# UNC-CFD/somar

Measured on AMD Instinct MI355X. Metric: pressure-Poisson V-cycles/sec, higher is better.
Workload: dtype f64; 1 GPU; C2 single-level 512^3 Poisson, diagonal stretched metric, Neumann, LevelGSRB V-cycle 2/2/2 + BiCGStab bottom; layout = 1 box(es) 512x512x512, one per GPU; mg_depth=8, cells=134217728

## Files before the change

### somar_amd/csrc/gsrb_fused.hip

```cpp
#include <type_traits>

#include "common.h"
#include "kernels.h"
#include "stencil_point.h"

namespace somar {


template <class T>
__device__ __forceinline__ typename Vec2<T>::type uni2(double c, bool, bool) { return mk2<T>(T(c), T(c)); }

template <int FR_J, int INMODE, bool DIRI, bool UNI, bool INT, int CLS, class T>
__device__ __forceinline__ void gsrb_fused_body(T* __restrict__ S, const Tile& t, const PatchDesc& p,
                                                T* __restrict__ phi_out,
                                                const T* __restrict__ phi_in,
                                                const T* __restrict__ rhs,
                                                const T* __restrict__ jgx,
                                                const T* __restrict__ jgy,
                                                const T* __restrict__ jgz,
                                                const T* __restrict__ jinv, const StencilParams& P,
                                                const double* __restrict__ sums,
                                                const PatchDesc* __restrict__ cpatches,
                                                const T* __restrict__ crse, int r0, int r1, int r2)
{
    typedef typename Vec2<T>::type T2;
    const T avg = (INMODE == 2 || INMODE == 4) ? T(sums[0] / sums[1]) : T(0);
    constexpr int LPR = 64 >> CLS;
    constexpr int NR = FR_J << CLS;
    constexpr int PITCH = 2 * LPR + (CLS >= 2 ? 2 : 0);
#define Sx(slot, r, c) S[((slot) * NR + (r)) * PITCH + (c)]
    const int lane = CLS == 0 ? (int)threadIdx.x : (int)(threadIdx.x & (LPR - 1));
    const int row = CLS == 0 ? (int)threadIdx.y
                             : (int)(((threadIdx.y >> 1) << (CLS + 1)) + (threadIdx.y & 1) + 2 * (threadIdx.x >> (6 - CLS)));
    const int ri = 2 * lane;
    const int li = t.i0 - 2 + ri;
    const int wi = t.w > 0 ? t.w : 2 * LPR - 4;
    const int lj = t.j0 - 2 + row;
    long long cbase = 0, cpk = 0, coff = 0;
    int cstep = 0, csh2 = 0;
    if (INMODE >= 3) {
        const PatchDesc cp = cpatches[t.patch];
        auto fdiv = [](int a, int b) { return a >= 0 ? a / b : -((-a + b - 1) / b); };
        const int ci0 = fdiv(li, r0);
        cstep = fdiv(li + 1, r0) - ci0;
        coff = cp.off;
        cbase = cp.off + ci0 + (long long)cp.pj * fdiv(lj, r1);
        cpk = cp.pk;
        csh2 = r2 >> 1;
    }
    auto ldphi = [&](int kp, bool ok0, bool ok1) {
        if (INMODE == 1) return mk2<T>(T(0), T(0));
        T2 v = ld2(phi_in, p.off + li + (long long)p.pj * lj + p.pk * kp, ok0, ok1, p.off);
        if (INMODE >= 3) {
            const bool any = ok0 || ok1;
            const long long c = any ? cbase + cpk * (long long)(kp >> csh2) : coff;
            const long long c2 = any ? c + cstep : coff;
            const T c0 = crse[c];
            const T c1 = crse[c2];
            v.x = ok0 ? v.x + c0 : T(0);
            v.y = ok1 ? v.y + c1 : T(0);
        }
        if (INMODE == 2 || INMODE == 4) { v.x = v.x - avg; v.y = v.y - avg; }
        return v;
    };
    const int gj = p.lo[1] + lj;
    const T xxS = T(1.0) / (T(P.dx[0]) * T(P.dx[0]));
    const T yyS = T(1.0) / (T(P.dx[1]) * T(P.dx[1]));
    const T zzS = T(1.0) / (T(P.dx[2]) * T(P.dx[2]));

    const bool fj = (lj >= -FRAME) && (lj < p.n[1] + FRAME);
    const bool fjh = (lj + 1 >= -FRAME) && (lj + 1 < p.n[1] + FRAME);
    const bool f0 = fj && (li >= -FRAME) && (li < p.n[0] + FRAME) && (ri < wi + 4);
    const bool f1 = fj && (li + 1 >= -FRAME) && (li + 1 < p.n[0] + FRAME) && (ri + 1 < wi + 4);
    const bool cf = (row >= 1) && (row <= NR - 2);
    const bool c0 = f0 && cf, c1 = f1 && cf;
    bool comp_ij[2], out_ij[2];
#pragma unroll
    for (int s = 0; s < 2; ++s) {
        const int l = li + s, g = p.lo[0] + l, r = ri + s;
        bool cmp = (l >= -1) && (l <= p.n[0]) && (r >= 1) && (r <= wi + 2) && (lj >= -1) && (lj <= p.n[1]) &&
                   (row >= 1) && (row <= NR - 2);
        if (!INT) {
            if ((g < P.dom_lo[0] && (P.neum[0][0] || (DIRI && P.diri[0][0]))) ||
                (g > P.dom_hi[0] && (P.neum[0][1] || (DIRI && P.diri[0][1]))))
                cmp = false;
            if ((gj < P.dom_lo[1] && (P.neum[1][0] || (DIRI && P.diri[1][0]))) ||
                (gj > P.dom_hi[1] && (P.neum[1][1] || (DIRI && P.diri[1][1]))))
                cmp = false;
            if ((l < 0 && (p.cf & 1)) || (l >= p.n[0] && (p.cf & 2))) cmp = false;
            if ((lj < 0 && (p.cf & 4)) || (lj >= p.n[1] && (p.cf & 8))) cmp = false;
        }
        comp_ij[s] = cmp;
        out_ij[s] = (l >= 0) && (l < p.n[0]) && (lj >= 0) && (lj < p.n[1]) && (r >= 2) && (r < wi + 2) &&
                    (row >= 2) && (row < NR - 2);
    }
    const long long sj = p.pj, sk = p.pk;
    const long long base = p.off + li + sj * lj;

    int k = t.k0 - 1;
    bool fk = (k - 1 >= -FRAME) && (k - 1 < p.n[2] + FRAME);
    T2 Pm = ldphi(k - 1, f0 && fk, f1 && fk);
    fk = (k >= -FRAME) && (k < p.n[2] + FRAME);
    T2 Pc = ldphi(k, f0 && fk, f1 && fk);
    T2 Gzc = UNI ? uni2<T>(P.uc[2], c0 && fk, c1 && fk) : ld2(jgz, base + sk * k, c0 && fk, c1 && fk, p.off);
    T b_rhs = 0, b_ji = 1, b_gxl = 0, b_gxh = 0, b_gyl = 0, b_gyh = 0, b_gzl = 0;
    T redPrev1 = 0, redPrev2 = 0;
    T2 Pn = mk2<T>(T(0), T(0)), Rn = mk2<T>(T(0), T(0));
    if (UNI) {
        const bool fkp0 = (k + 1 >= -FRAME) && (k + 1 < p.n[2] + FRAME);
        Pn = ldphi(k + 1, f0 && fkp0, f1 && fkp0);
        Rn = ld2(rhs, base + sk * k, c0 && fk, c1 && fk, p.off);
    }

    const int kend = t.k0 + t.nk;
    auto step = [&](auto CC) {
        constexpr int c = decltype(CC)::value;
        const int gk = p.lo[2] + k;
        fk = (k >= -FRAME) && (k < p.n[2] + FRAME);
        const bool fkp = (k + 1 >= -FRAME) && (k + 1 < p.n[2] + FRAME);
        T2 Pp, Rh;
        if (UNI) {
            Pp = Pn;
            Rh = Rn;
            const bool fkpp = (k + 2 >= -FRAME) && (k + 2 < p.n[2] + FRAME);
            Pn = ldphi(k + 2, f0 && fkpp, f1 && fkpp);
            Rn = ld2(rhs, base + sk * (k + 1), c0 && fkp, c1 && fkp, p.off);
        } else {
            Pp = ldphi(k + 1, f0 && fkp, f1 && fkp);
            Rh = ld2(rhs, base + sk * k, c0 && fk, c1 && fk, p.off);
        }
        const T2 Gzp = UNI ? uni2<T>(P.uc[2], c0 && fkp, c1 && fkp) : ld2(jgz, base + sk * (k + 1), c0 && fkp, c1 && fkp, p.off);
        const T2 Ji = UNI ? uni2<T>(P.uc[3], c0 && fk, c1 && fk) : ld2(jinv, base + sk * k, c0 && fk, c1 && fk, p.off);
        const T2 Gx = UNI ? uni2<T>(P.uc[0], c0 && fk, c1 && fk) : ld2(jgx, base + sk * k, c0 && fk, c1 && fk, p.off);
        const T2 Gy = UNI ? uni2<T>(P.uc[1], c0 && fk, c1 && fk) : ld2(jgy, base + sk * k, c0 && fk, c1 && fk, p.off);
        const T2 Gyh = UNI ? uni2<T>(P.uc[1], c0 && fk && fjh, c1 && fk && fjh)
                           : ld2(jgy, base + sk * k + sj, c0 && fk && fjh, c1 && fk && fjh, p.off);
        const T gx_next = __shfl_down(Gx.x, 1, 64);

        const int slot = ((k % 3) + 3) % 3;
        *reinterpret_cast<T2*>(&Sx(slot, row, ri)) = Pc;
        __syncthreads();

        const int rc = ri + c;
        T red = pick<T>(Pc, c);
        {
            bool comp = comp_ij[c] && (k >= -1) && (k <= p.n[2]);
            if ((gk < P.dom_lo[2] && (P.neum[2][0] || (DIRI && P.diri[2][0]))) ||
                (gk > P.dom_hi[2] && (P.neum[2][1] || (DIRI && P.diri[2][1]))))
                comp = false;
            if ((k < 0 && (p.cf & 16)) || (k >= p.n[2] && (p.cf & 32))) comp = false;
            if (comp) {
                const T pxl = Sx(slot, row, rc - 1), pxh = Sx(slot, row, rc + 1);
                const T pyl = Sx(slot, row - 1, rc), pyh = Sx(slot, row + 1, rc);
                red = gsrb_point<DIRI, INT, T>(P, xxS, yyS, zzS, p.lo[0] + li + c, gj, gk, pxl, pxh, pyl, pyh, pick<T>(Pm, c),
                                 pick<T>(Pp, c), c ? Gx.y : Gx.x, c ? gx_next : Gx.y, pick<T>(Gy, c), pick<T>(Gyh, c),
                                 pick<T>(Gzc, c), pick<T>(Gzp, c), pick<T>(Ji, c), pick<T>(Rh, c), red);
                Sx(slot, row, rc) = red;
            }
        }

        {
            const int kb = k - 1;
            if ((kb >= t.k0) && (kb < t.k0 + t.nk) && (out_ij[0] || out_ij[1])) {
                const int sb = ((kb % 3) + 3) % 3;
                T black = 0;
                if (out_ij[c]) {
                    T pxl = Sx(sb, row, rc - 1), pxh = Sx(sb, row, rc + 1);
                    T pyl = Sx(sb, row - 1, rc), pyh = Sx(sb, row + 1, rc);
                    T pzl = redPrev2, pzh = red;
                    if (INT ? (p.cf & 48) != 0 : p.cf != 0) {
                        const T own = Sx(sb, row, rc);
                        const int l = li + c;
                        const T xl = pxl, xh = pxh, yl = pyl, yh = pyh, zl = pzl, zh = pzh;
                        if (!INT) {
                            if ((p.cf & 1) && l == 0) pxl = T(P.cf_c1[0]) * own + T(P.cf_c2[0]) * xh;
                            if ((p.cf & 2) && l == p.n[0] - 1) pxh = T(P.cf_c1[0]) * own + T(P.cf_c2[0]) * xl;
                            if ((p.cf & 4) && lj == 0) pyl = T(P.cf_c1[1]) * own + T(P.cf_c2[1]) * yh;
                            if ((p.cf & 8) && lj == p.n[1] - 1) pyh = T(P.cf_c1[1]) * own + T(P.cf_c2[1]) * yl;
                        }
                        if ((p.cf & 16) && kb == 0) pzl = T(P.cf_c1[2]) * own + T(P.cf_c2[2]) * zh;
                        if ((p.cf & 32) && kb == p.n[2] - 1) pzh = T(P.cf_c1[2]) * own + T(P.cf_c2[2]) * zl;
                    }
                    black = gsrb_point<DIRI, INT, T>(P, xxS, yyS, zzS, p.lo[0] + li + c, gj, p.lo[2] + kb, pxl, pxh, pyl, pyh,
                                       pzl, pzh, b_gxl, b_gxh, b_gyl, b_gyh, b_gzl, pick<T>(Gzc, c), b_ji, b_rhs,
                                       Sx(sb, row, rc));
                }
                T* dst = phi_out + base + sk * kb;
                const T ox = c ? redPrev1 : black, oy = c ? black : redPrev1;
                if (out_ij[0] && out_ij[1]) *reinterpret_cast<T2*>(dst) = mk2<T>(ox, oy);
                else if (out_ij[0]) dst[0] = ox;
                else dst[1] = oy;
            }
        }

        {
            const int cb = c ^ 1;
            b_rhs = pick<T>(Rh, cb);
            b_ji = pick<T>(Ji, cb);
            b_gxl = cb ? Gx.y : Gx.x;
            b_gxh = cb ? gx_next : Gx.y;
            b_gyl = pick<T>(Gy, cb);
            b_gyh = pick<T>(Gyh, cb);
            b_gzl = pick<T>(Gzc, cb);
        }
        redPrev2 = redPrev1;
        redPrev1 = red;
        Pm = Pc;
        Pc = Pp;
        Gzc = Gzp;
    };
    const int cfirst = __builtin_amdgcn_readfirstlane((p.lo[0] + li + gj + p.lo[2] + k) & 1);
    if (cfirst) {
        for (;;) {
            if (k > kend) break;
            step(std::integral_constant<int, 1>{});
            ++k;
            if (k > kend) break;
            step(std::integral_constant<int, 0>{});
            ++k;
        }
    } else {
        for (;;) {
            if (k > kend) break;
            step(std::integral_constant<int, 0>{});
            ++k;
            if (k > kend) break;
            step(std::integral_constant<int, 1>{});
            ++k;
        }
    }
#undef Sx
}

template <int FR_J, int INMODE, bool DIRI = false, bool UNI = false, int NARROW = 0, class T = double>
__global__ __launch_bounds__(64 * FR_J) void k_gsrb_fused(const Tile* __restrict__ tiles,
                                                     const PatchDesc* __restrict__ patches,
                                                     T* __restrict__ phi_out,
                                                     const T* __restrict__ phi_in,
                                                     const T* __restrict__ rhs,
                                                     const T* __restrict__ jgx,
                                                     const T* __restrict__ jgy,
                                                     const T* __restrict__ jgz,
                                                     const T* __restrict__ jinv, StencilParams P,
                                                     const double* __restrict__ sums,
                                                     const PatchDesc* __restrict__ cpatches,
                                                     const T* __restrict__ crse, int r0, int r1, int r2, int lean_ok)
{
    __shared__ __attribute__((aligned(16))) T S[3 * FR_J * (NARROW == 1 ? 160 : 128)];
    const Tile t = tiles[blockIdx.x];
    const PatchDesc p = patches[t.patch];
    const int cls = NARROW == 1 ? t.cls : (NARROW == 2 ? 1 : 0);
    bool lean = false;
    if (UNI && !DIRI) {
        const int wi = t.w > 0 ? t.w : 124;
        const int ilo = t.i0 - 1, ihi = min(t.i0 + wi, p.n[0]), jlo = t.j0 - 1, jhi = min(t.j0 + (FR_J << cls) - 4, p.n[1]);
        lean = lean_ok && p.lo[0] + ilo > P.dom_lo[0] && p.lo[0] + ihi < P.dom_hi[0] && p.lo[1] + jlo > P.dom_lo[1] &&
               p.lo[1] + jhi < P.dom_hi[1] && !((p.cf & 1) && ilo < 0) && !((p.cf & 2) && ihi >= p.n[0]) &&
               !((p.cf & 4) && jlo < 0) && !((p.cf & 8) && jhi >= p.n[1]);
    }
#define SOMAR_FUSED_BODY(INT_, CLS_)                                                                                          \
    gsrb_fused_body<FR_J, INMODE, DIRI, UNI, INT_, CLS_, T>(S, t, p, phi_out, phi_in, rhs, jgx, jgy, jgz, jinv, P, sums, cpatches, \
                                                        crse, r0, r1, r2)
    if constexpr (NARROW == 2) {
        SOMAR_FUSED_BODY(false, 1);
    } else if (!NARROW || cls == 0) {
        if (lean) SOMAR_FUSED_BODY(UNI && !DIRI, 0);
        else SOMAR_FUSED_BODY(false, 0);
    } else if (cls == 1) {
        if (lean) SOMAR_FUSED_BODY(UNI && !DIRI, NARROW ? 1 : 0);
        else SOMAR_FUSED_BODY(false, NARROW ? 1 : 0);
    } else {
        SOMAR_FUSED_BODY(false, NARROW ? 4 : 0);
    }
#undef SOMAR_FUSED_BODY
}

template <class T>
static void launch_gsrb_fused_t(hipStream_t st, TileSpan tiles, const LevelDev& L, const MetricPtrs<T>& M,
                                T* phi_out, const T* phi_in, const T* rhs, int in_mode, const double* sums,
                                const LevelDev* C, const T* crse, const int* r)
{
    if (tiles.n == 0) return;
    const PatchDesc* cpatches = C ? C->patches : nullptr;
    const int r0 = r ? r[0] : 1, r1 = r ? r[1] : 1, r2 = r ? r[2] : 1;
    SOMAR_CHECK(in_mode < 3 || ((r0 == 1 || r0 == 2) && (r1 == 1 || r1 == 2) && (r2 == 1 || r2 == 2)),
                "internal: the prolongation folded into a sweep takes multigrid ratios of 1 or 2 per direction");
    auto go = [&](auto kern, int rows) {
        hipLaunchKernelGGL(kern, dim3(tiles.n), dim3(64, rows, 1), 0, st, tiles.p, L.patches, phi_out, phi_in, rhs, M.jg[0], M.jg[1],
                           M.jg[2], M.jinv, L.P, sums, cpatches, crse, r0, r1, r2, L.lean_tiles);
    };
#define SOMAR_FUSED_MODES(ROWS, D, U, N, M0, M1, M2, M3, M4)                    \
    switch (in_mode) {                                                          \
        case 1: go(k_gsrb_fused<ROWS, M1, D, U, N, T>, ROWS); break;            \
        case 2: go(k_gsrb_fused<ROWS, M2, D, U, N, T>, ROWS); break;            \
        case 3: go(k_gsrb_fused<ROWS, M3, D, U, N, T>, ROWS); break;            \
        case 4: go(k_gsrb_fused<ROWS, M4, D, U, N, T>, ROWS); break;            \
        default: go(k_gsrb_fused<ROWS, M0, D, U, N, T>, ROWS);                  \
    }
    const bool rows16 = L.fused_rows == 16;
    const bool narrow = tiles.classes != 0 && rows16;
    const bool tall = tiles.classes == 2;
    SOMAR_CHECK(!tall || (rows16 && !L.P.uniform), "internal: tall tiles on a level whose fused sweep has no class-1 kernel");
    bool diri = false;
    for (int d = 0; d < 3; ++d) diri = diri || L.P.diri[d][0] || L.P.diri[d][1];
    if (diri) {
        SOMAR_CHECK(in_mode == 0 || in_mode == 1 || in_mode == 3, "internal: mean removal on a level with Dirichlet sides");
        if (!rows16) { SOMAR_FUSED_MODES(8, true, false, false, 0, 1, 0, 3, 3) }
        else if (tall) { SOMAR_FUSED_MODES(16, true, false, 2, 0, 1, 0, 3, 3) }
        else if (narrow) { SOMAR_FUSED_MODES(16, true, false, true, 0, 1, 0, 3, 3) }
        else { SOMAR_FUSED_MODES(16, true, false, false, 0, 1, 0, 3, 3) }
        return;
    }
    if (L.P.uniform && rows16) {
        if (narrow) { SOMAR_FUSED_MODES(16, false, true, true, 0, 1, 2, 3, 4) }
        else { SOMAR_FUSED_MODES(16, false, true, false, 0, 1, 2, 3, 4) }
        return;
    }
    if (!rows16) { SOMAR_FUSED_MODES(8, false, false, false, 0, 1, 2, 3, 4) }
    else if (tall) { SOMAR_FUSED_MODES(16, false, false, 2, 0, 1, 2, 3, 4) }
    else if (narrow) { SOMAR_FUSED_MODES(16, false, false, true, 0, 1, 2, 3, 4) }
    else { SOMAR_FUSED_MODES(16, false, false, false, 0, 1, 2, 3, 4) }
#undef SOMAR_FUSED_MODES
}

void launch_gsrb_fused(hipStream_t st, TileSpan tiles, const LevelDev& L, const MetricPtrs<double>& M,
                       double* phi_out, const double* phi_in, const double* rhs, int in_mode, const double* sums,
                       const LevelDev* C, const double* crse, const int* r)
{
    launch_gsrb_fused_t<double>(st, tiles, L, M, phi_out, phi_in, rhs, in_mode, sums, C, crse, r);
}

void launch_gsrb_fused(hipStream_t st, TileSpan tiles, const LevelDev& L, const MetricPtrs<float>& M,
                       float* phi_out, const float* phi_in, const float* rhs, int in_mode, const double* sums,
                       const LevelDev* C, const float* crse, const int* r)
{
    SOMAR_CHECK(fused_uniform_kernel(L) || (M.jg[0] && M.jg[1] && M.jg[2] && M.jinv),
                "internal: the fused sweep streams the metric of this depth, but its fp32 copies are missing");
    launch_gsrb_fused_t<float>(st, tiles, L, M, phi_out, phi_in, rhs, in_mode, sums, C, crse, r);
}

bool fused_uniform_kernel(const LevelDev& L)
{
    bool diri = false;
    for (int d = 0; d < 3; ++d) diri = diri || L.P.diri[d][0] || L.P.diri[d][1];
    return L.P.uniform && L.fused_rows == 16 && !diri;
}

}
```

### somar_amd/csrc/kernels.h

```cpp
#pragma once
#include "common.h"

namespace somar {

struct TileSpan {
    const Tile* p = nullptr;
    int n = 0;
    int classes = 0;
};

struct LevelDev {
    const Tile* tiles = nullptr;
    int ntiles = 0;
    int tile_j = 4;
    const CopyItem* tile_items = nullptr;
    const int* tile_item_start = nullptr;
    int ghost_gy = 16;
    const PatchDesc* patches = nullptr;
    int npatches = 0;
    double* jg[3] = {nullptr, nullptr, nullptr};
    double* jinv = nullptr;
    double* lapdiag = nullptr;
    double* jgf[3][3] = {{nullptr, nullptr, nullptr}, {nullptr, nullptr, nullptr}, {nullptr, nullptr, nullptr}};
    StencilParams P;
    const double* bc_face = nullptr;
    int fused_rows = 16;
    int full_rows = 8;
    int lean_tiles = 1;
    int ordered_serial = 0;
};

template <class T>
struct MetricPtrs { const T* jg[3]; const T* jinv; };
inline MetricPtrs<double> metric_ptrs(const LevelDev& L) { return MetricPtrs<double>{{L.jg[0], L.jg[1], L.jg[2]}, L.jinv}; }

struct FullFlux { const double* psi = nullptr; const double* J[3][3] = {{nullptr, nullptr, nullptr}, {nullptr, nullptr, nullptr}, {nullptr, nullptr, nullptr}}; double dxi[3] = {0, 0, 0}; };

void launch_ghost_ops(hipStream_t st, const LevelDev& L, const GhostOp* ops, int nops, double* phi, double* psi,
                      bool bc_homog = true, bool redirect = false);
void launch_ghost_ops(hipStream_t st, const LevelDev& L, const GhostOp* ops, int nops, float* phi);
void launch_ghost_program(hipStream_t st, const LevelDev& L, const GhostOp* box_ops, const int* box_first, double* phi,
                          double* psi, bool bc_homog, bool redirect, bool copy_all);
void launch_full_march(hipStream_t st, TileSpan tiles, const LevelDev& L, double* out, const double* phi,
                       const double* psi, const double* rhs, int mode);
void launch_gsrb_full_march(hipStream_t st, TileSpan tiles, const LevelDev& L, double* out,
                            const double* phi, const double* psi, const double* rhs, int color);
void launch_full_fused(hipStream_t st, TileSpan tiles, const LevelDev& L, double* out, const double* phi,
                       const double* psi, const double* rhs);
void launch_gsrb_full_shell(hipStream_t st, TileSpan tiles, const LevelDev& L, double* phi, const double* phi_in,
                            const double* psi, const double* rhs);
void launch_flux_full(hipStream_t st, const LevelDev& L, double* const out[3], const double* phi, const double* psi);
void launch_op_full(hipStream_t st, const LevelDev& L, double* out, const double* phi, const double* psi,
                    const double* rhs, int mode);
void launch_gsrb_full(hipStream_t st, const LevelDev& L, double* phi, const double* psi, const double* rhs, int color);

void launch_gsrb_ortho(hipStream_t st, const LevelDev& L, double* phi, const double* rhs, int color, int loose = 0,
                       bool pull = false);
void launch_gsrb_fused(hipStream_t st, TileSpan tiles, const LevelDev& L, const MetricPtrs<double>& M,
                       double* phi_out, const double* phi_in, const double* rhs, int in_mode, const double* sums,
                       const LevelDev* C, const double* crse, const int* r);
void launch_gsrb_fused(hipStream_t st, TileSpan tiles, const LevelDev& L, const MetricPtrs<float>& M,
                       float* phi_out, const float* phi_in, const float* rhs, int in_mode, const double* sums,
                       const LevelDev* C, const float* crse, const int* r);
bool fused_uniform_kernel(const LevelDev& L);
void launch_resid_march(hipStream_t st, TileSpan tiles, const LevelDev& L, double* out,
                        const double* phi, const double* rhs, int mode);
void launch_resid_restrict(hipStream_t st, TileSpan tiles, const LevelDev& F, const MetricPtrs<double>& M,
                           const LevelDev& C, double* crse, const double* phi, const double* rhs, const int r[3],
                           double dxProduct, double* volsum);
void launch_resid_restrict(hipStream_t st, TileSpan tiles, const LevelDev& F, const MetricPtrs<float>& M,
                           const LevelDev& C, float* crse, const float* phi, const float* rhs, const int r[3],
                           double dxProduct, double* volsum);
template <int NF>
struct SweepFields { double* out[NF]; const double* in[NF]; const double* rhs[NF]; };
template <int NF>
struct FieldOps { StencilParams P[NF]; };
template <int NF, class OPS>
void launch_gsrb_fused_nf(hipStream_t st, TileSpan tiles, const LevelDev& L, const SweepFields<NF>& F, const OPS& O, int in_mode);
template <int NF>
struct ResidFields { double* out[NF]; const double* phi[NF]; const double* rhs[NF]; };
template <int NF, class OPS>
void launch_resid_nf(hipStream_t st, TileSpan tiles, const LevelDev& F, const ResidFields<NF>& fields, const OPS& O,
                     const LevelDev* C, const int* r);
void launch_child_volume(hipStream_t st, const LevelDev& C, const LevelDev& F, double* crse, const int r[3],
                         double dxProduct);
void launch_sum_partials(hipStream_t st, const double* partials, int n, double* out);
void launch_combine_sums(hipStream_t st, double* out, const double* a, const double* b, const double* c);
void launch_line_gsrb_2d(hipStream_t st, const LevelDev& L, int maxN0, double* phi, const double* rhs, double* dmod, int color,
                         const double* psi);
void launch_line_gsrb_ortho(hipStream_t st, TileSpan ctiles, int tile_j, const LevelDev& L,
                            double* phi, const double* rhs, double* dmod, int color, const double* psi = nullptr);
void launch_op_ortho(hipStream_t st, const LevelDev& L, double* out, const double* phi, const double* rhs, int mode,
                     bool pull = false);
void launch_lapdiag(hipStream_t st, const LevelDev& L);
void launch_diag(hipStream_t st, const LevelDev& L, double* phi, const double* r, int mode);
void launch_restrict(hipStream_t st, const LevelDev& C, const LevelDev& F, double* crse, const double* fine,
                     const int r[3]);
void launch_prolong(hipStream_t st, const LevelDev& F, const LevelDev& C, double* fine, const double* crse,
                    const int r[3], bool zeroAvg, double dxProduct, double* partials, double* sums,
                    long long fieldElems, bool ordered = false);
void launch_sub_mean(hipStream_t st, double* f, long long n, const double* sums);
void launch_avg_harmonic(hipStream_t st, const LevelDev& C, const LevelDev& F, double* crse, const double* fine,
                         const int r[3]);
void launch_avg_face(hipStream_t st, const LevelDev& C, const LevelDev& F, int patch, const int cn[3], double* crse,
                     const double* fine, int dir, const int r[3]);
void launch_copy_items(hipStream_t st, const LevelDev& L, const CopyItem* items, int nitems, double* f);
void launch_copy_items(hipStream_t st, const LevelDev& L, const CopyItem* items, int nitems, float* f);
void launch_pack(hipStream_t st, const LevelDev& L, const CopyItem* items, const long long* bufoff, int nitems,
                 double* f, double* buf, bool pack);
void launch_pack(hipStream_t st, const LevelDev& L, const CopyItem* items, const long long* bufoff, int nitems,
                 float* f, float* buf, bool pack);
// ... 118 lines not shown
```

### somar_amd/csrc/level.cpp

```cpp
#include "level.h"
#include "march_plan.h"

#include <algorithm>
#include <array>
#include <cstdlib>
#include <cstring>

namespace somar {

bool coarsenable(const std::vector<IBox>& boxes, const int* r)
{
    for (const IBox& b : boxes)
        if (!(b.coarsen(r).refine(r) == b)) return false;
    return true;
}

ExchangePlan build_exchange_plan(const IBox& domain, const bool periodic[3], const int ghost[3],
                                 const std::vector<IBox>& boxes, const std::vector<int>& owner, int myrank)
{
    ExchangePlan plan;
    std::vector<std::array<int, 3>> shifts;
    for (int a = -1; a <= 1; ++a)
        for (int b = -1; b <= 1; ++b)
            for (int cc = -1; cc <= 1; ++cc) {
// ... 431 lines not shown
void Level::build_march_tiles(const MarchRequest& req)
{
    namespace mp = march_plan;
    march = req;
    ftiles.clear(); rtiles.clear(); qtiles.clear(); gtiles.clear(); stiles.clear();
    std::vector<mp::BoxSize> sizes;
    for (const PatchDesc& p : hpatches) sizes.push_back({p.n[0], p.n[1], p.n[2]});
    auto tuned = [&](mp::Shape s) {
        s.classes = s.classes && !tune.no_narrow_tiles;
        s.balanced = !tune.no_balanced_tiles;
        return s;
    };
    const bool tall = req.tall7 && !tune.no_narrow_tiles && tune.narrow_7pt != 0 &&
                      mp::tall_eligible(sizes, dev.fused_rows, dev.P.uniform != 0);
    const mp::Shape fshape = tuned(mp::fused_shape(dev.fused_rows, req.narrow7)), rshape = tuned(mp::resid_shape(req.narrow7));
    mp::Table f = mp::march_tiles(fshape, sizes, tall), r = mp::march_tiles(rshape, sizes);
    mp::number_slots(r.tiles);
    mp::Table q = mp::march_tiles(tuned(mp::full_shape(dev.full_rows)), sizes);
    if (!plan.peers.empty()) {
        std::vector<mp::Region> recv;
        for (const CopyItem& it : plan.recv_items)
            recv.push_back({it.dst_patch, {it.dst_lo[0], it.dst_lo[1], it.dst_lo[2]}, {it.n[0], it.n[1], it.n[2]}});
        auto split = [&](SplitTileTable& t, const mp::Table& all, const mp::Shape& shape, int halo) {
            std::vector<Tile> own, rem;
            mp::split(all.tiles, shape, halo, sizes, recv, own, rem);
            t.own.assign(std::move(own), all.classes);
            t.rem.assign(std::move(rem), all.classes);
        };
        split(ftiles, f, fshape, FRAME);
        split(rtiles, r, rshape, 1);
    }
    ftiles.all.assign(std::move(f.tiles), f.classes);
    rtiles.all.assign(std::move(r.tiles), r.classes);
    qtiles.assign(std::move(q.tiles), q.classes);
    if (req.fused19) {
        mp::Table g = mp::march_tiles(tuned(mp::fused19_shape()), sizes), sh = mp::shell_tiles(sizes);
        gtiles.assign(std::move(g.tiles), g.classes);
        stiles.assign(std::move(sh.tiles), sh.classes);
    }
}

void Level::define(const IBox& dom, const bool per[3], const double dx_[3], const int bct[3][2],
                   const std::vector<IBox>& bx, const std::vector<int>& own, Comm* c, const Tuning& t)
{
    domain = dom;
    comm = c;
    tune = t;
    dev.fused_rows = (int)t.fused_rows;
    dev.full_rows = (int)t.full_rows;
    dev.lean_tiles = t.no_lean_tiles ? 0 : 1;
    dev.ordered_serial = t.ordered_serial ? 1 : 0;
    const int myrank = c ? c->rank : 0;
    for (int d = 0; d < 3; ++d) {
        periodic[d] = per[d];
        dx[d] = dx_[d];
        bc_type[d][0] = bct[d][0];
        bc_type[d][1] = bct[d][1];
    }
    boxes = bx;
    owner = own;
    if (owner.empty()) owner.assign(boxes.size(), 0);
    SOMAR_CHECK(owner.size() == boxes.size(), "owner/box count mismatch");

    local.clear();
    hpatches.clear();
    long long cursor = 0;
    valid_cells_global = 0;
    for (size_t b = 0; b < boxes.size(); ++b) {
        SOMAR_CHECK(!boxes[b].empty(), "empty box in layout");
        valid_cells_global += boxes[b].numPts();
        if (owner[b] != myrank) continue;
        PatchDesc p;
        std::memset(&p, 0, sizeof(p));
        for (int d = 0; d < 3; ++d) { p.lo[d] = boxes[b].lo[d]; p.n[d] = boxes[b].size(d); }
        p.pj = ((p.n[0] + 2 * FRAME + 1) / 2) * 2;
        p.pk = (long long)p.pj * (p.n[1] + 2 * FRAME);
        const long long elems = p.pk * (p.n[2] + 2 * FRAME);
        p.off = cursor + FRAME * p.pk + (long long)FRAME * p.pj + FRAME;
        cursor += ((elems + 31) / 32) * 32;
        hpatches.push_back(p);
        local.push_back((int)b);
    }
    field_elems = cursor;

    int tj = TILE_J_MAX, tk = TILE_K_MAX;
    auto count_tiles = [&](int tj_, int tk_) {
        long long c = 0;
        for (const PatchDesc& p : hpatches)
            c += (long long)((p.n[0] + TILE_I - 1) / TILE_I) * ((p.n[1] + tj_ - 1) / tj_) * ((p.n[2] + tk_ - 1) / tk_);
        return c;
    };
    while (count_tiles(tj, tk) < 1024 && tk > 1) tk /= 2;
    while (count_tiles(tj, tk) < 1024 && tj > 1) tj /= 2;
    dev.tile_j = tj;
    std::vector<Tile> nat;
    for (int pi = 0; pi < (int)hpatches.size(); ++pi) {
        const PatchDesc& p = hpatches[pi];
        for (int k0 = 0; k0 < p.n[2]; k0 += tk)
            for (int j0 = 0; j0 < p.n[1]; j0 += tj)
                for (int i0 = 0; i0 < p.n[0]; i0 += TILE_I)
                    nat.push_back(march_plan::make_tile(pi, i0, j0, k0, std::min(tk, p.n[2] - k0), 0, 0));
    }
    const int N = (int)nat.size();

    {
        std::vector<Tile> ct;
        for (int pi = 0; pi < (int)hpatches.size(); ++pi) {
            const PatchDesc& p = hpatches[pi];
            for (int j0 = 0; j0 < p.n[1]; j0 += ctile_j)
                for (int i0 = 0; i0 < p.n[0]; i0 += TILE_I) ct.push_back(march_plan::make_tile(pi, i0, j0, 0, p.n[2], 0, 0));
        }
        ctiles.assign(std::move(ct), 0);
    }

    int ghost[3];
    for (int d = 0; d < 3; ++d) ghost[d] = active[d] ? FRAME : 0;
    plan = build_exchange_plan(domain, periodic, ghost, boxes, owner, myrank);
    {
        std::vector<int> patch_of(boxes.size(), -1);
        for (int pi = 0; pi < (int)local.size(); ++pi) patch_of[local[pi]] = pi;
        for (CopyItem& it : plan.local) { it.src_patch = patch_of[it.src_patch]; it.dst_patch = patch_of[it.dst_patch]; }
        for (CopyItem& it : plan.send_items) it.src_patch = patch_of[it.src_patch];
        for (CopyItem& it : plan.recv_items) it.dst_patch = patch_of[it.dst_patch];
    }

    d_patches = DevBuf<PatchDesc>::from(hpatches);
    tiles.assign(march_plan::xcd_order(nat), 0);
    d_local_items = DevBuf<CopyItem>::from(plan.local);
    d_send_items = DevBuf<CopyItem>::from(plan.send_items);
    d_recv_items = DevBuf<CopyItem>::from(plan.recv_items);
    d_send_off = DevBuf<long long>::from(plan.send_itemoff);
    d_recv_off = DevBuf<long long>::from(plan.recv_itemoff);
    build_march_tiles(MarchRequest{false, false, march.fused19});
    d_sendbuf = plan.send_total ? DevBuf<double>(plan.send_total) : DevBuf<double>();
    d_recvbuf = plan.recv_total ? DevBuf<double>(plan.recv_total) : DevBuf<double>();

    dev.tiles = tiles.span().p;
    dev.ntiles = N;
    dev.patches = d_patches;
    dev.npatches = (int)hpatches.size();
    {
        const long long pullMax = tune.pull_max_cells;
        long long cells = 0;
        for (const IBox& b : boxes) cells += b.numPts();
        if (plan.peers.empty() && cells <= pullMax && N > 0) {
            std::vector<std::vector<int>> byDst(hpatches.size());
            for (int q = 0; q < (int)plan.local.size(); ++q) byDst[plan.local[q].dst_patch].push_back(q);
            std::vector<CopyItem> titems;
            std::vector<int> tstart(N + 1, 0);
            for (int b = 0; b < N; ++b) {
                const Tile& t = tiles.host()[b];
                const PatchDesc& p = hpatches[t.patch];
                int lo[3] = {t.i0, t.j0, t.k0};
                int hi[3] = {std::min(t.i0 + TILE_I, p.n[0]) - 1, std::min(t.j0 + dev.tile_j, p.n[1]) - 1, t.k0 + t.nk - 1};
                for (int d = 0; d < 3; ++d)
                    if (active[d]) { lo[d] -= 1; hi[d] += 1; }
                tstart[b] = (int)titems.size();
                for (int q : byDst[t.patch]) {
                    const CopyItem& it = plan.local[q];
                    CopyItem c = it;
                    bool empty = false;
                    for (int d = 0; d < 3; ++d) {
                        const int a = std::max(lo[d], it.dst_lo[d]), e = std::min(hi[d], it.dst_lo[d] + it.n[d] - 1);
                        if (e < a) { empty = true; break; }
                        c.dst_lo[d] = a;
                        c.src_lo[d] = it.src_lo[d] + (a - it.dst_lo[d]);
// ... 314 lines not shown
```

### somar_amd/csrc/tuning.cpp

```cpp
#include "tuning.h"

#include <cstdlib>
#include <cstring>
#include <string>

namespace somar {

namespace {
enum Rule {
    PRESENT,
    NONZERO,
    COUNT,
    INT,
    ONLY,
};
struct Switch { const char* name; long long Tuning::*field; Rule rule; int alt; };
const Switch SWITCHES[] = {
    {"FUSED_MIN_CELLS", &Tuning::fused_min_cells, COUNT, 0},
    {"MARCH_MIN_CELLS", &Tuning::march_min_cells, COUNT, 0},
    {"FUSED_ROWS", &Tuning::fused_rows, ONLY, 8},
    {"FULL_ROWS", &Tuning::full_rows, ONLY, 6},
    {"NO_BALANCED_TILES", &Tuning::no_balanced_tiles, PRESENT, 0},
    {"NO_NARROW_TILES", &Tuning::no_narrow_tiles, PRESENT, 0},
    {"NARROW_7PT", &Tuning::narrow_7pt, NONZERO, 0},
    {"NO_LEAN_TILES", &Tuning::no_lean_tiles, PRESENT, 0},
    {"NO_UNIFORM", &Tuning::no_uniform, NONZERO, 0},
    {"NO_ZERO_PLANES", &Tuning::no_zero_planes, NONZERO, 0},
    {"NO_ZERO_START", &Tuning::no_zero_start, PRESENT, 0},
    {"NO_FOLD_PROLONG", &Tuning::no_fold_prolong, PRESENT, 0},
    {"NO_CF_FUSED", &Tuning::no_cf_fused, PRESENT, 0},
    {"AMR_PLAIN", &Tuning::amr_plain, NONZERO, 0},
    {"FUSED_BOTTOM_MAX_CELLS", &Tuning::fused_bottom_max_cells, COUNT, 0},
    {"BOX_BOTTOM", &Tuning::box_bottom, NONZERO, 0},
    {"BOX_BOTTOM_MIN_CELLS", &Tuning::box_bottom_min_cells, COUNT, 0},
    {"BOX_TIMING", &Tuning::box_timing, PRESENT, 0},
    {"BOTTOM_ASYNC", &Tuning::bottom_async, NONZERO, 0},
    {"ORDERED_REDUCE_MAX", &Tuning::ordered_reduce_max, COUNT, 0},
    {"ORDERED_SERIAL", &Tuning::ordered_serial, PRESENT, 0},
    {"NO_FUSED_PUBLISH", &Tuning::no_fused_publish, PRESENT, 0},
    {"POLL_FETCH", &Tuning::poll_fetch, NONZERO, 0},
    {"GHOST_STAGED", &Tuning::ghost_staged, NONZERO, 0},
    {"NO_GHOST_DCE", &Tuning::no_ghost_dce, PRESENT, 0},
    {"FLUX_FIELDS", &Tuning::flux_fields, PRESENT, 0},
    {"FUSED19_MIN_BOX", &Tuning::fused19_min_box, INT, 0},
    {"CF_FULL_GATHER", &Tuning::cf_full_gather, PRESENT, 0},
    {"PULL_MAX_CELLS", &Tuning::pull_max_cells, COUNT, 0},
    {"GRAPH_CELLS", &Tuning::graph_cells, COUNT, 0},
    {"AGGLOM_CELLS", &Tuning::agglom_cells, COUNT, 0},
    {"NO_OVERLAP", &Tuning::no_overlap, NONZERO, 0},
    {"TIMING", &Tuning::timing, INT, 0},
};
}

Tuning Tuning::from_env()
{
    Tuning t;
    bool march_set = false;
    for (const Switch& s : SWITCHES) {
        const char* e = getenv((std::string("SOMAR_") + s.name).c_str());
        if (!e) continue;
        long long& v = t.*s.field;
        switch (s.rule) {
            case PRESENT: v = 1; break;
            case NONZERO: v = atoi(e) != 0; break;
            case COUNT: v = atoll(e); break;
            case INT: v = atoi(e); break;
            case ONLY: if (atoi(e) == s.alt) v = s.alt; break;
        }
        if (s.field == &Tuning::march_min_cells) march_set = true;
    }
    if (!march_set) t.march_min_cells = t.fused_min_cells;
    return t;
}

bool Tuning::get(const char* name, long long* value) const
{
    for (const Switch& s : SWITCHES)
        if (!strcmp(name, s.name)) { *value = this->*s.field; return true; }
    return false;
}

}
```

### somar_amd/csrc/tuning.h

```cpp
#pragma once

namespace somar {

struct Tuning {
    long long fused_min_cells = 262144;
    long long march_min_cells = 262144;
    long long fused_rows = 16;
    long long full_rows = 8;
    long long no_balanced_tiles = 0;
    long long no_narrow_tiles = 0;
    long long narrow_7pt = -1;
    long long no_lean_tiles = 0;
    long long no_uniform = 0;
    long long no_zero_planes = 0;
    long long no_zero_start = 0;
    long long no_fold_prolong = 0;
    long long no_cf_fused = 0;
    long long amr_plain = 0;
    long long fused_bottom_max_cells = 512;
    long long box_bottom = 1;
    long long box_bottom_min_cells = 513;
    long long box_timing = 0;
    long long bottom_async = 1;
    long long ordered_reduce_max = 4096;
    long long ordered_serial = 0;
    long long no_fused_publish = 0;
    long long poll_fetch = 1;
    long long ghost_staged = 0;
    long long no_ghost_dce = 0;
    long long flux_fields = 0;
    long long fused19_min_box = -1;
    long long cf_full_gather = 0;
    long long pull_max_cells = 262144;
    long long graph_cells = 262144;
    long long agglom_cells = 2097152;
    long long no_overlap = 0;
    long long timing = 0;

    static Tuning from_env();
    bool get(const char* name, long long* value) const;
};

}
```

Before: 103.8 V-cycles/s.

## Stage metric coefficients into LDS with async global_load_lds one plane ahead

Adds a staged variant of the fused GSRB kernel for fp64 16-row non-uniform tiles. The six coefficient streams (rhs, jinv, jgx, jgy, the jgy row above, jgz of the next plane) are prefetched one k-plane ahead straight into per-wave LDS buffers with global_load_lds, and phi for the next plane is loaded raw one step early. This aims to hide global memory latency behind the current plane's compute. In exchange it uses more LDS, which may lower occupancy, and relies on hand-placed waitcnt instructions. It is on by default for levels with at least 4M cells.

```diff
diff --git a/somar_amd/csrc/gsrb_fused.hip b/somar_amd/csrc/gsrb_fused.hip
--- a/somar_amd/csrc/gsrb_fused.hip
+++ b/somar_amd/csrc/gsrb_fused.hip
@@ -10,8 +10,28 @@
 template <class T>
 __device__ __forceinline__ typename Vec2<T>::type uni2(double c, bool, bool) { return mk2<T>(T(c), T(c)); }
 
-template <int FR_J, int INMODE, bool DIRI, bool UNI, bool INT, int CLS, class T>
-__device__ __forceinline__ void gsrb_fused_body(T* __restrict__ S, const Tile& t, const PatchDesc& p,
+constexpr int STG_STREAMS = 6;
+constexpr bool STAGED_MODES[5] = {true, true, true, false, false};
+constexpr bool STAGED_MODES_MIXED[5] = {false, true, false, false, false};
+template <class T>
+__device__ __forceinline__ void stage2(const T* __restrict__ safe, long long rel, bool ok0, bool ok1, T* wave_slot)
+{
+    static_assert(sizeof(T) == 8, "a staged pair is one 16-byte load: fp64 only");
+    __builtin_amdgcn_global_load_lds((const __attribute__((address_space(1))) void*)(safe + ((ok0 || ok1) ? rel : 0LL)),
+                                     (__attribute__((address_space(3))) void*)wave_slot, 16, 0, 0);
+}
+__device__ __forceinline__ double wave_uniform(double x)
+{
+    return __hiloint2double(__builtin_amdgcn_readfirstlane(__double2hiint(x)), __builtin_amdgcn_readfirstlane(__double2loint(x)));
+}
+template <class T>
+__device__ __forceinline__ typename Vec2<T>::type sel2(const typename Vec2<T>::type& v, bool ok0, bool ok1)
+{
+    return mk2<T>(ok0 ? v.x : T(0), ok1 ? v.y : T(0));
+}
+
+template <int FR_J, int INMODE, bool DIRI, bool UNI, bool INT, int CLS, bool STG, class T>
+__device__ __forceinline__ void gsrb_fused_body(T* __restrict__ S, T* __restrict__ G, const Tile& t, const PatchDesc& p,
                                                 T* __restrict__ phi_out,
                                                 const T* __restrict__ phi_in,
                                                 const T* __restrict__ rhs,
@@ -24,15 +44,18 @@
                                                 const T* __restrict__ crse, int r0, int r1, int r2)
 {
     typedef typename Vec2<T>::type T2;
-    const T avg = (INMODE == 2 || INMODE == 4) ? T(sums[0] / sums[1]) : T(0);
+    T avg = (INMODE == 2 || INMODE == 4) ? T(sums[0] / sums[1]) : T(0);
+    if constexpr (STG) avg = wave_uniform(avg);
     constexpr int LPR = 64 >> CLS;
     constexpr int NR = FR_J << CLS;
     constexpr int PITCH = 2 * LPR + (CLS >= 2 ? 2 : 0);
-#define Sx(slot, r, c) S[((slot) * NR + (r)) * PITCH + (c)]
+#define Sx(slot, r, c) \
+    (*(STG ? &Sp[(slot) * (NR * PITCH) + ((r) - row) * PITCH + ((c) - ri)] : &S[((slot) * NR + (r)) * PITCH + (c)]))
     const int lane = CLS == 0 ? (int)threadIdx.x : (int)(threadIdx.x & (LPR - 1));
     const int row = CLS == 0 ? (int)threadIdx.y
                              : (int)(((threadIdx.y >> 1) << (CLS + 1)) + (threadIdx.y & 1) + 2 * (threadIdx.x >> (6 - CLS)));
     const int ri = 2 * lane;
+    T* const Sp = S + row * PITCH + ri;
     const int li = t.i0 - 2 + ri;
     const int wi = t.w > 0 ? t.w : 2 * LPR - 4;
     const int lj = t.j0 - 2 + row;
@@ -63,10 +86,37 @@
         if (INMODE == 2 || INMODE == 4) { v.x = v.x - avg; v.y = v.y - avg; }
         return v;
     };
+    struct RawPhi { T2 v; T c0, c1; };
+    auto ldphi_raw = [&](int kp, bool ok0, bool ok1) {
+        RawPhi w;
+        w.v = mk2<T>(T(0), T(0));
+        w.c0 = w.c1 = T(0);
+        if (INMODE == 1) return w;
+        const bool any = ok0 || ok1;
+        w.v = *reinterpret_cast<const T2*>(phi_in + (any ? p.off + li + (long long)p.pj * lj + p.pk * kp : p.off));
+        if (INMODE >= 3) {
+            const long long c = any ? cbase + cpk * (long long)(kp >> csh2) : coff;
+            const long long c2 = any ? c + cstep : coff;
+            w.c0 = crse[c];
+            w.c1 = crse[c2];
+        }
+        return w;
+    };
+    auto ldphi_use = [&](const RawPhi& w, bool ok0, bool ok1) {
+        if (INMODE == 1) return mk2<T>(T(0), T(0));
+        T2 v = sel2<T>(w.v, ok0, ok1);
+        if (INMODE >= 3) {
+            v.x = ok0 ? v.x + w.c0 : T(0);
+            v.y = ok1 ? v.y + w.c1 : T(0);
+        }
+        if (INMODE == 2 || INMODE == 4) { v.x = v.x - avg; v.y = v.y - avg; }
+        return v;
+    };
     const int gj = p.lo[1] + lj;
-    const T xxS = T(1.0) / (T(P.dx[0]) * T(P.dx[0]));
-    const T yyS = T(1.0) / (T(P.dx[1]) * T(P.dx[1]));
-    const T zzS = T(1.0) / (T(P.dx[2]) * T(P.dx[2]));
+    T xxS = T(1.0) / (T(P.dx[0]) * T(P.dx[0]));
+    T yyS = T(1.0) / (T(P.dx[1]) * T(P.dx[1]));
+    T zzS = T(1.0) / (T(P.dx[2]) * T(P.dx[2]));
+    if constexpr (STG) { xxS = wave_uniform(xxS); yyS = wave_uniform(yyS); zzS = wave_uniform(zzS); }
 
     const bool fj = (lj >= -FRAME) && (lj < p.n[1] + FRAME);
     const bool fjh = (lj + 1 >= -FRAME) && (lj + 1 < p.n[1] + FRAME);
@@ -96,6 +146,7 @@
     }
     const long long sj = p.pj, sk = p.pk;
     const long long base = p.off + li + sj * lj;
+    const int rel0 = li + p.pj * lj;
 
     int k = t.k0 - 1;
     bool fk = (k - 1 >= -FRAME) && (k - 1 < p.n[2] + FRAME);
@@ -111,6 +162,30 @@
         Pn = ldphi(k + 1, f0 && fkp0, f1 && fkp0);
         Rn = ld2(rhs, base + sk * k, c0 && fk, c1 && fk, p.off);
     }
+    const int wave = __builtin_amdgcn_readfirstlane((int)threadIdx.y);
+#define GW(s) (G + (wave * STG_STREAMS + (s)) * 128)
+#define GL(s) (*reinterpret_cast<const T2*>(GW(s) + 2 * (int)threadIdx.x))
+    auto stage = [&](int kk) {
+        const bool gk0 = (kk >= -FRAME) && (kk < p.n[2] + FRAME) && (kk <= t.k0 + t.nk);
+        const bool gk1 = (kk + 1 >= -FRAME) && (kk + 1 < p.n[2] + FRAME) && (kk <= t.k0 + t.nk);
+        if constexpr (STG) {
+            const long long rel = rel0 + sk * kk;
+            stage2(rhs + p.off, rel, c0 && gk0, c1 && gk0, GW(0));
+            stage2(jinv + p.off, rel, c0 && gk0, c1 && gk0, GW(1));
+            stage2(jgx + p.off, rel, c0 && gk0, c1 && gk0, GW(2));
+            stage2(jgy + p.off, rel, c0 && gk0, c1 && gk0, GW(3));
+            stage2(jgy + p.off, rel + sj, c0 && gk0 && fjh, c1 && gk0 && fjh, GW(4));
+            stage2(jgz + p.off, rel + sk, c0 && gk1, c1 && gk1, GW(5));
+        }
+    };
+    RawPhi Pr;
+    Pr.v = mk2<T>(T(0), T(0));
+    Pr.c0 = Pr.c1 = T(0);
+    if constexpr (STG) {
+        const bool fkp0 = (k + 1 >= -FRAME) && (k + 1 < p.n[2] + FRAME);
+        stage(k);
+        Pr = ldphi_raw(k + 1, f0 && fkp0, f1 && fkp0);
+    }
 
     const int kend = t.k0 + t.nk;
     auto step = [&](auto CC) {
@@ -118,7 +193,9 @@
         const int gk = p.lo[2] + k;
         fk = (k >= -FRAME) && (k < p.n[2] + FRAME);
         const bool fkp = (k + 1 >= -FRAME) && (k + 1 < p.n[2] + FRAME);
-        T2 Pp, Rh;
+        T2 Pp, Rh, Gzp, Ji, Gx, Gy, Gyh;
+        T gx_next;
+        if constexpr (!STG) {
         if (UNI) {
             Pp = Pn;
             Rh = Rn;
@@ -129,17 +206,32 @@
             Pp = ldphi(k + 1, f0 && fkp, f1 && fkp);
             Rh = ld2(rhs, base + sk * k, c0 && fk, c1 && fk, p.off);
         }
-        const T2 Gzp = UNI ? uni2<T>(P.uc[2], c0 && fkp, c1 && fkp) : ld2(jgz, base + sk * (k + 1), c0 && fkp, c1 && fkp, p.off);
-        const T2 Ji = UNI ? uni2<T>(P.uc[3], c0 && fk, c1 && fk) : ld2(jinv, base + sk * k, c0 && fk, c1 && fk, p.off);
-        const T2 Gx = UNI ? uni2<T>(P.uc[0], c0 && fk, c1 && fk) : ld2(jgx, base + sk * k, c0 && fk, c1 && fk, p.off);
-        const T2 Gy = UNI ? uni2<T>(P.uc[1], c0 && fk, c1 && fk) : ld2(jgy, base + sk * k, c0 && fk, c1 && fk, p.off);
-        const T2 Gyh = UNI ? uni2<T>(P.uc[1], c0 && fk && fjh, c1 && fk && fjh)
+        Gzp = UNI ? uni2<T>(P.uc[2], c0 && fkp, c1 && fkp) : ld2(jgz, base + sk * (k + 1), c0 && fkp, c1 && fkp, p.off);
+        Ji = UNI ? uni2<T>(P.uc[3], c0 && fk, c1 && fk) : ld2(jinv, base + sk * k, c0 && fk, c1 && fk, p.off);
+        Gx = UNI ? uni2<T>(P.uc[0], c0 && fk, c1 && fk) : ld2(jgx, base + sk * k, c0 && fk, c1 && fk, p.off);
+        Gy = UNI ? uni2<T>(P.uc[1], c0 && fk, c1 && fk) : ld2(jgy, base + sk * k, c0 && fk, c1 && fk, p.off);
+        Gyh = UNI ? uni2<T>(P.uc[1], c0 && fk && fjh, c1 && fk && fjh)
                            : ld2(jgy, base + sk * k + sj, c0 && fk && fjh, c1 && fk && fjh, p.off);
-        const T gx_next = __shfl_down(Gx.x, 1, 64);
+        gx_next = __shfl_down(Gx.x, 1, 64);
+        }
 
         const int slot = ((k % 3) + 3) % 3;
         *reinterpret_cast<T2*>(&Sx(slot, row, ri)) = Pc;
         __syncthreads();
+        if constexpr (STG) {
+            Pp = ldphi_use(Pr, f0 && fkp, f1 && fkp);
+            Rh = sel2<T>(GL(0), c0 && fk, c1 && fk);
+            Ji = sel2<T>(GL(1), c0 && fk, c1 && fk);
+            Gx = sel2<T>(GL(2), c0 && fk, c1 && fk);
+            Gy = sel2<T>(GL(3), c0 && fk, c1 && fk);
+            Gyh = sel2<T>(GL(4), c0 && fk && fjh, c1 && fk && fjh);
+            Gzp = sel2<T>(GL(5), c0 && fkp, c1 && fkp);
+            asm volatile("s_waitcnt lgkmcnt(0)" ::: "memory");
+            const bool fkpp = (k + 2 >= -FRAME) && (k + 2 < p.n[2] + FRAME);
+            stage(k + 1);
+            Pr = ldphi_raw(k + 2, f0 && fkpp, f1 && fkpp);
+            gx_next = __shfl_down(Gx.x, 1, 64);
+        }
 
         const int rc = ri + c;
         T red = pick<T>(Pc, c);
@@ -185,7 +277,7 @@
                                        pzl, pzh, b_gxl, b_gxh, b_gyl, b_gyh, b_gzl, pick<T>(Gzc, c), b_ji, b_rhs,
                                        Sx(sb, row, rc));
                 }
-                T* dst = phi_out + base + sk * kb;
+                T* dst = STG ? phi_out + p.off + (rel0 + sk * kb) : phi_out + base + sk * kb;
                 const T ox = c ? redPrev1 : black, oy = c ? black : redPrev1;
                 if (out_ij[0] && out_ij[1]) *reinterpret_cast<T2*>(dst) = mk2<T>(ox, oy);
                 else if (out_ij[0]) dst[0] = ox;
@@ -229,10 +321,13 @@
             ++k;
         }
     }
+    if constexpr (STG) asm volatile("s_waitcnt vmcnt(0)" ::: "memory");
+#undef GL
+#undef GW
 #undef Sx
 }
 
-template <int FR_J, int INMODE, bool DIRI = false, bool UNI = false, int NARROW = 0, class T = double>
+template <int FR_J, int INMODE, bool DIRI = false, bool UNI = false, int NARROW = 0, class T = double, bool STG = false>
 __global__ __launch_bounds__(64 * FR_J) void k_gsrb_fused(const Tile* __restrict__ tiles,
                                                      const PatchDesc* __restrict__ patches,
                                                      T* __restrict__ phi_out,
@@ -247,6 +342,8 @@
                                                      const T* __restrict__ crse, int r0, int r1, int r2, int lean_ok)
 {
     __shared__ __attribute__((aligned(16))) T S[3 * FR_J * (NARROW == 1 ? 160 : 128)];
+    __shared__ __attribute__((aligned(16))) T G[STG ? STG_STREAMS * FR_J * 128 : 2];
+    static_assert(!STG || (FR_J == 16 && !UNI && sizeof(T) == 8), "staged coefficients: the fp64 streamed 16-row kernels");
     const Tile t = tiles[blockIdx.x];
     const PatchDesc p = patches[t.patch];
     const int cls = NARROW == 1 ? t.cls : (NARROW == 2 ? 1 : 0);
@@ -259,7 +356,7 @@
                !((p.cf & 4) && jlo < 0) && !((p.cf & 8) && jhi >= p.n[1]);
     }
 #define SOMAR_FUSED_BODY(INT_, CLS_)                                                                                          \
-    gsrb_fused_body<FR_J, INMODE, DIRI, UNI, INT_, CLS_, T>(S, t, p, phi_out, phi_in, rhs, jgx, jgy, jgz, jinv, P, sums, cpatches, \
+    gsrb_fused_body<FR_J, INMODE, DIRI, UNI, INT_, CLS_, STG, T>(S, G, t, p, phi_out, phi_in, rhs, jgx, jgy, jgz, jinv, P, sums, cpatches, \
                                                         crse, r0, r1, r2)
     if constexpr (NARROW == 2) {
         SOMAR_FUSED_BODY(false, 1);
@@ -276,6 +373,12 @@
 }
 
 template <class T>
+constexpr bool staged_mode(int rows, bool uni, int narrow, int in_mode)
+{
+    return sizeof(T) == 8 && rows == 16 && !uni && (narrow == 1 ? STAGED_MODES_MIXED[in_mode] : STAGED_MODES[in_mode]);
+}
+
+template <class T>
 static void launch_gsrb_fused_t(hipStream_t st, TileSpan tiles, const LevelDev& L, const MetricPtrs<T>& M,
                                 T* phi_out, const T* phi_in, const T* rhs, int in_mode, const double* sums,
                                 const LevelDev* C, const T* crse, const int* r)
@@ -285,17 +388,23 @@
     const int r0 = r ? r[0] : 1, r1 = r ? r[1] : 1, r2 = r ? r[2] : 1;
     SOMAR_CHECK(in_mode < 3 || ((r0 == 1 || r0 == 2) && (r1 == 1 || r1 == 2) && (r2 == 1 || r2 == 2)),
                 "internal: the prolongation folded into a sweep takes multigrid ratios of 1 or 2 per direction");
-    auto go = [&](auto kern, int rows) {
-        hipLaunchKernelGGL(kern, dim3(tiles.n), dim3(64, rows, 1), 0, st, tiles.p, L.patches, phi_out, phi_in, rhs, M.jg[0], M.jg[1],
-                           M.jg[2], M.jinv, L.P, sums, cpatches, crse, r0, r1, r2, L.lean_tiles);
-    };
+    auto go = [&](auto kern0, auto kern1, int rows) {
+        auto launch = [&](auto kern) {
+            hipLaunchKernelGGL(kern, dim3(tiles.n), dim3(64, rows, 1), 0, st, tiles.p, L.patches, phi_out, phi_in, rhs, M.jg[0],
+                               M.jg[1], M.jg[2], M.jinv, L.P, sums, cpatches, crse, r0, r1, r2, L.lean_tiles);
+        };
+        if (L.staged_coef) launch(kern1);
+        else launch(kern0);
+    };
+#define SOMAR_FUSED_KERN(ROWS, D, U, N, M) \
+    k_gsrb_fused<ROWS, M, D, U, N, T>, k_gsrb_fused<ROWS, M, D, U, N, T, staged_mode<T>(ROWS, U, N, M)>
 #define SOMAR_FUSED_MODES(ROWS, D, U, N, M0, M1, M2, M3, M4)                    \
     switch (in_mode) {                                                          \
-        case 1: go(k_gsrb_fused<ROWS, M1, D, U, N, T>, ROWS); break;            \
-        case 2: go(k_gsrb_fused<ROWS, M2, D, U, N, T>, ROWS); break;            \
-        case 3: go(k_gsrb_fused<ROWS, M3, D, U, N, T>, ROWS); break;            \
-        case 4: go(k_gsrb_fused<ROWS, M4, D, U, N, T>, ROWS); break;            \
-        default: go(k_gsrb_fused<ROWS, M0, D, U, N, T>, ROWS);                  \
+        case 1: go(SOMAR_FUSED_KERN(ROWS, D, U, N, M1), ROWS); break;           \
+        case 2: go(SOMAR_FUSED_KERN(ROWS, D, U, N, M2), ROWS); break;           \
+        case 3: go(SOMAR_FUSED_KERN(ROWS, D, U, N, M3), ROWS); break;           \
+        case 4: go(SOMAR_FUSED_KERN(ROWS, D, U, N, M4), ROWS); break;           \
+        default: go(SOMAR_FUSED_KERN(ROWS, D, U, N, M0), ROWS);                 \
     }
     const bool rows16 = L.fused_rows == 16;
     const bool narrow = tiles.classes != 0 && rows16;
@@ -321,6 +430,7 @@
     else if (narrow) { SOMAR_FUSED_MODES(16, false, false, true, 0, 1, 2, 3, 4) }
     else { SOMAR_FUSED_MODES(16, false, false, false, 0, 1, 2, 3, 4) }
 #undef SOMAR_FUSED_MODES
+#undef SOMAR_FUSED_KERN
 }
 
 void launch_gsrb_fused(hipStream_t st, TileSpan tiles, const LevelDev& L, const MetricPtrs<double>& M,
diff --git a/somar_amd/csrc/kernels.h b/somar_amd/csrc/kernels.h
--- a/somar_amd/csrc/kernels.h
+++ b/somar_amd/csrc/kernels.h
@@ -27,6 +27,7 @@
     int fused_rows = 16;
     int full_rows = 8;
     int lean_tiles = 1;
+    int staged_coef = 0;
     int ordered_serial = 0;
 };
 
diff --git a/somar_amd/csrc/level.cpp b/somar_amd/csrc/level.cpp
--- a/somar_amd/csrc/level.cpp
+++ b/somar_amd/csrc/level.cpp
@@ -537,6 +537,7 @@
         local.push_back((int)b);
     }
     field_elems = cursor;
+    dev.staged_coef = !t.no_staged_coef && valid_cells_global >= t.staged_min_cells ? 1 : 0;
 
     int tj = TILE_J_MAX, tk = TILE_K_MAX;
     auto count_tiles = [&](int tj_, int tk_) {
diff --git a/somar_amd/csrc/tuning.cpp b/somar_amd/csrc/tuning.cpp
--- a/somar_amd/csrc/tuning.cpp
+++ b/somar_amd/csrc/tuning.cpp
@@ -70,6 +70,8 @@
         if (s.field == &Tuning::march_min_cells) march_set = true;
     }
     if (!march_set) t.march_min_cells = t.fused_min_cells;
+    if (const char* e = getenv("SOMAR_NO_STAGED_COEF")) t.no_staged_coef = atoi(e) != 0;
+    if (const char* e = getenv("SOMAR_STAGED_MIN_CELLS")) t.staged_min_cells = atoll(e);
     return t;
 }
 
@@ -77,6 +79,8 @@
 {
     for (const Switch& s : SWITCHES)
         if (!strcmp(name, s.name)) { *value = this->*s.field; return true; }
+    if (!strcmp(name, "NO_STAGED_COEF")) { *value = no_staged_coef; return true; }
+    if (!strcmp(name, "STAGED_MIN_CELLS")) { *value = staged_min_cells; return true; }
     return false;
 }
 
diff --git a/somar_amd/csrc/tuning.h b/somar_amd/csrc/tuning.h
--- a/somar_amd/csrc/tuning.h
+++ b/somar_amd/csrc/tuning.h
@@ -11,6 +11,8 @@
     long long no_narrow_tiles = 0;
     long long narrow_7pt = -1;
     long long no_lean_tiles = 0;
+    long long no_staged_coef = 0;
+    long long staged_min_cells = 4194304;
     long long no_uniform = 0;
     long long no_zero_planes = 0;
     long long no_zero_start = 0;
```

Result: faster. 105.9 V-cycles/s (median of 6 runs) (+2.0%).
